# tangtang888/video-edge-ai-proxy

Measured on AMD Instinct MI355X. Metric: decoded FPS (whole node) + p50 VideoLatestImage latency, 256×1080p RTSP, higher is better.
Workload: dtype uint8 (BGR24 frames; bf16-capable consumer path)

## Files before the change

### csrc/bind_ext.h

```cpp
#pragma once
#include <pybind11/pybind11.h>

void bind_net(pybind11::module_& m);
void bind_mux(pybind11::module_& m);
void bind_hevc(pybind11::module_& m);
void bind_bus(pybind11::module_& m);
void bind_rpc(pybind11::module_& m);
void bind_dbk(pybind11::module_& m);
void bind_hevc_lf(pybind11::module_& m);
```

### csrc/bindings.cpp

```cpp
#include <malloc.h>

#include <pybind11/numpy.h>
#include <pybind11/pybind11.h>
#include <pybind11/stl.h>

#include "vep/hostprof.h"
#include "vep/avc.h"
#include "vep/avc_cavlc.h"
#include "vep/avc_recon.h"
#include "vep/bench_driver.h"
#include "vep/cabac.h"
#include "vep/codec.h"
#include "vep/gpu.h"
#include "vep/h264.h"
#include "vep/hevc_ctu.h"
#include "vep/hevc_dec.h"
#include "vep/hevc_kern.h"
#include "vep/jpeg.h"
#include "vep/scale.h"
#include "bind_ext.h"
#include "vep/runtime.h"
#include "vep/synth.h"

namespace py = pybind11;
// ... 2464 lines not shown
  m.def("letterbox_geometry", [](int src_w, int src_h, int size, bool even) {
    gpu::LetterboxDesc d{};
    d.src_w = src_w;
    d.src_h = src_h;
    gpu::fill_letterbox_geometry(d, size, even);
    return py::make_tuple(d.nw, d.nh, d.pad_x, d.pad_y);
  }, py::arg("src_w"), py::arg("src_h"), py::arg("size"), py::arg("even") = false);

  bind_net(m);
  bind_mux(m);
  bind_hevc(m);
  bind_bus(m);
  bind_rpc(m);
  bind_dbk(m);
  bind_hevc_lf(m);
}
```

### csrc/vep/avc.cpp

```cpp
#include "avc.h"

#include <immintrin.h>

#include <algorithm>
#include <array>

#include "avc_cavlc.h"
#include "avc_internal.h"
#include "fanout.h"

namespace vep::avc {

using h264::Pps;
using h264::Sps;


void MbNeighbours::reset(int wmbs, int hmbs, bool ring) {
  w_ = wmbs;
  h_ = hmbs;
  cur_ = -1;
  run_slice_ = ~0u;
  run_start_ = 0;
  announced_ = 0;
  const size_t n = size_t(wmbs) * hmbs;
// ... 1487 lines not shown
  if (par) {
    const int W = pic->wmbs, H = pic->hmbs;
    ColMotion* col_target = colb.col;
    FanOut::shared().run(nunits, [&](int k) {
      SliceUnit& u = *units_[size_t(k)];
      u.nb.reset(W, H, true);
      Picture& sh = u.shard;
      sh.wmbs = W;
      sh.hmbs = H;
      if (sh.mbs.size() != size_t(W) * H) sh.mbs.assign(size_t(W) * H, MbRec{});
      sh.coefs.clear();
      sh.mvs.clear();
      sh.wps.clear();
      sh.intra_mbs = sh.intra_res = sh.inter_mbs = 0;
      sh.deblock = false;
      sh.target = pic->target;
      sh.dpb_slots = pic->dpb_slots;
      sh.constrained_intra = pic->constrained_intra;
      sh.poc = pic->poc;
      sh.bd = pic->bd;
      sh.cf = pic->cf;
      sh.qp_bias = pic->qp_bias;
      sh.qpc_bias = pic->qpc_bias;
      u.colb.col = col_target;
      u.colb.set_uids(&u.uids);
      sh.colb = col_target ? &u.colb : nullptr;
      parse_slice_data(u.nb, sh, u.sh, *u.sps, *u.pps, u.rbsp.data(), u.rbsp.size(), u.bitpos, u.slice_idx, u.list);
#if defined(__x86_64__)
      _mm_sfence();
#endif
    });
    parallel_slices_run_ += u64(nunits);
    covered.assign(size_t(pic->nmbs()), 0);
    for (int k = 0; k < nunits; ++k) {
      SliceUnit& u = *units_[size_t(k)];
      const Picture& sh = u.shard;
      const u32 coef0 = u32(pic->coefs.size()), mv0 = u32(pic->mvs.size()), wp0 = u32(pic->wps.size());
      const u32 res0 = u32(pic->intra_res);
      pic->coefs.insert(pic->coefs.end(), sh.coefs.begin(), sh.coefs.end());
      pic->mvs.insert(pic->mvs.end(), sh.mvs.begin(), sh.mvs.end());
      pic->wps.insert(pic->wps.end(), sh.wps.begin(), sh.wps.end());
      pic->intra_mbs += sh.intra_mbs;
      pic->intra_res += sh.intra_res;
      pic->inter_mbs += sh.inter_mbs;
      pic->deblock |= sh.deblock;
      for (int mb = u.sh.first_mb; mb < pic->nmbs(); ++mb) {
        if (!u.nb.announced(mb)) continue;
        VEP_CHECK(!covered[size_t(mb)], "H.264: slices overlap");
        covered[size_t(mb)] = 1;
        MbRec m = sh.mbs[size_t(mb)];
        m.coef += coef0;
        if (m.kind == kSkip || m.kind == kInter) m.mv += mv0;
        if (m.flags & kMbWp) m.wp += wp0;
        if (m.res != kNoRes) m.res += res0;
        pic->mbs[size_t(mb)] = m;
      }
    }
  }
  int ncovered = 0;
  if (par)
// ... 19 lines not shown
      }
      for (auto& rf : m.ref) rf = u8(cs);
      m.mv = u32(pic->mvs.size());
      m.flags |= kMbMv16;
      pic->mvs.resize(pic->mvs.size() + 2, 0);
      ++pic->inter_mbs;
    } else {
      m.kind = kI16x16;
      m.i16_mode = 2;
      std::fill(std::begin(m.ref), std::end(m.ref), u8(0xFF));
      ++pic->intra_mbs;
    }
  }
  pic->info.coded_mbs = pic->nmbs() - missing;
  const u32 uid = next_uid_++;
  if (first.field_pic) {
    if (first.nal_ref_idc != 0)
      mark_field(first, *act_sps, pic->target >> 1, pic->poc, uid, second_field && pair_.ref, std::move(col_built));
    if (first.has_mmco5() && !second_field) {
      pic->poc = 0;
      pair_.frame_num = 0;
      pair_.poc[int(first.bottom_field)] = 0;
      pair_.boundary = true;
      pair_.hard = reorder_cur_ == 0;
    }
    if (second_field) close_pair(*pic);
  } else {
    if (first.nal_ref_idc != 0) {
      mark_references(first, *act_sps, pic->target, pic->poc, uid, std::move(col_built));
    }
// ... 41 lines not shown
      more = br.pos() < stop;
      ++mb;
    }
    return;
  }
  SliceEnv env;
  env.sh = &sh;
  env.sps = &sps;
  env.pps = &pps;
  env.slice = slice_idx;
  env.list[0] = &lists[0];
  env.list[1] = &lists[1];
  env.cur_poc = pic.poc;
  env.scaling = h264::resolve_scaling(sps, pps);
  env.field = sh.field_pic;
  decode_slice_generic(nb, pic, env, data, n, bitpos);
}

static inline void validate_mb(const Picture& p, const MbRec& m, bool written = false) {
  const size_t ncoef = p.coefs.size(), nmv = p.mvs.size();
  VEP_CHECK(m.kind <= kI8x8, "macroblock kind out of range");
  VEP_CHECK(p.cf == 2 || m.chroma_coded < 0x100, "chroma block mask out of range");
  VEP_CHECK(m.qp <= 51 + p.qp_bias && m.qpc <= 51 + p.qpc_bias && m.qpc2 <= 51 + p.qpc_bias,
            "macroblock QP out of range");
  if (m.kind == kIPcm) {
    const size_t ns = p.cf == 2 ? size_t(kPcmMaxSamples) : size_t(kPcmMbBytes);
    VEP_CHECK(size_t(m.coef) + (p.bd > 8 ? ns : ns / 2) <= ncoef, "I_PCM samples outside the pool");
    return;
  }
  const size_t nw = size_t(coef_words(m));
// ... 110 lines not shown
    stream_words(&col->b[size_t(mb) * 4], out, sizeof out);
    return;
  }
  ColMotion::Blk* out = &col->b[size_t(mb) * 16];
  for (int blk = 0; blk < 16; ++blk) {
    const int b8 = ((blk >> 3) << 1) | ((blk & 3) >> 1);
    const int l = st.ref[0][b8] >= 0 ? 0 : 1;
    const int ri = st.ref[l][b8];
    if (ri < 0) {
      out[blk] = ColMotion::Blk{{0, 0}, 0u, i8(-1)};
      continue;
    }
    out[blk] = ColMotion::Blk{{st.mv[l][blk][0], st.mv[l][blk][1]},
                              size_t(ri) < lu[size_t(l)].size() ? lu[size_t(l)][size_t(ri)] : 0u, i8(ri)};
  }
}

std::shared_ptr<ColMotion> build_col_motion(const MbNeighbours& nb, int wmbs, int hmbs,
                                            const std::vector<std::array<std::vector<u32>, 2>>& slice_uids,
                                            bool corners, Recycler<ColMotion>* pool) {
  auto col = pool ? pool->acquire([](ColMotion&) {}) : std::make_shared<ColMotion>();
  col->wmbs = wmbs;
  col->hmbs = hmbs;
  col->corners = corners;
  const int per = corners ? 4 : 16;
  col->b.resize(size_t(wmbs) * hmbs * size_t(per));
  static constexpr u8 kCorner[4] = {0, 3, 12, 15};
  for (int mb = 0; mb < wmbs * hmbs; ++mb) {
    const MbState& st = nb.at(mb);
    ColMotion::Blk* out = &col->b[size_t(mb) * size_t(per)];
// ... 237 lines not shown
  for (int l = 0; l < nl; ++l, out += per) {
    const i16* v = &s.mv[l][0][0];
    if (per == 2) {
      std::memcpy(out, v, 4);
    } else if (per == 8) {
      std::memcpy(out, v, 4);
      std::memcpy(out + 2, v + 4, 4);
      std::memcpy(out + 4, v + 16, 4);
      std::memcpy(out + 6, v + 20, 4);
    } else {
      std::memcpy(out, v, 64);
    }
  }
}

static inline void store_rec(MbRec* dst, const MbRec& m) {
  static_assert(sizeof(MbRec) % 8 == 0 && sizeof(ColMotion::Blk) * 4 % 8 == 0, "8-byte words");
  stream_words(dst, &m, sizeof(MbRec));
}

void store_skip_mb(Picture& pic, int mb, MbRec& m, const MbState& s) {
  m.coef = u32(pic.coefs.size());
  m.luma_coded = 0;
  m.chroma_coded = 0;
  m.wp = 0;
  m.res = kNoRes;
  store_motion(pic, m, s);
  ++pic.inter_mbs;
  if (!(m.dbk & 1)) pic.deblock = true;
  for (int k = 0; k < 4; ++k) {
    const int r0 = m.ref[k], r1 = m.ref1[k];
    VEP_CHECK((r0 != 0xFF || r1 != 0xFF) && (r0 == 0xFF || r0 < pic.dpb_slots) && (r1 == 0xFF || r1 < pic.dpb_slots) &&
                  (r1 == 0xFF || (m.flags & kMbL1)),
              "skipped macroblock reference slot outside the DPB");
  }
  VEP_CHECK(m.qp <= 51 + pic.qp_bias && m.qpc <= 51 + pic.qpc_bias && m.qpc2 <= 51 + pic.qpc_bias,
            "macroblock QP out of range");
  store_rec(&pic.mbs[size_t(mb)], m);
  if (pic.colb) pic.colb->store(mb, s);
}

void store_mb(Picture& pic, int mb, MbRec m, const MbState& s, const MbResidual* res, const u8* pcm,
              const WpEntry* wp) {
  m.coef = u32(pic.coefs.size());
  m.luma_coded = 0;
  m.chroma_coded = 0;
  if (m.kind == kIPcm) {
    VEP_CHECK(pcm, "I_PCM macroblock without samples");
    const size_t ns = pic.cf == 2 ? size_t(kPcmMaxSamples) : size_t(kPcmMbBytes);
    const size_t o = pic.coefs.size(), nb = pic.bd > 8 ? 2 * ns : ns;
    pic.coefs.resize(o + nb / 2);
    std::memcpy(pic.coefs.data() + o, pcm, nb);
  } else if (res && (res->luma | res->chroma)) {
    m.luma_coded = res->luma;
    m.chroma_coded = res->chroma;
    if (res->t8) m.flags |= kMbT8x8;
    const i16* grp[32];
    int ng = 0;
    if (res->t8) {
      for (int q = 0; q < 4; ++q)
        if ((res->luma >> ((q & 1) * 2 + (q >> 1) * 8)) & 1)
          for (int w = 0; w < 4; ++w) grp[ng++] = res->b8[q] + 16 * w;
    } else {
      for (u32 w = res->luma; w; w &= w - 1) grp[ng++] = res->blk[__builtin_ctz(w)];
    }
    for (u32 w = res->chroma; w; w &= w - 1) grp[ng++] = res->blk[16 + __builtin_ctz(w)];
    u16 mask[32];
    int nv = 0;
    for (int g = 0; g < ng; ++g) {
      mask[g] = nonzero_mask16(grp[g]);
      nv += __builtin_popcount(mask[g]);
    }
    const size_t o = pic.coefs.size();
    i16* out = pic.coefs.extend(size_t(ng + nv) + 8);
    std::memcpy(out, mask, size_t(ng) * sizeof(u16));
    i16* v = out + ng;
    for (int g = 0; g < ng; ++g) v = compact16(grp[g], mask[g], v);
    pic.coefs.resize(o + size_t(ng + nv));
  }
  m.mv = 0;
  m.wp = 0;
  m.flags &= u8(~(kMbMv8x8 | kMbMv16));
  if (m.kind == kSkip || m.kind == kInter) {
    store_motion(pic, m, s);
    if (wp && (m.flags & kMbWp)) {
      m.wp = u32(pic.wps.size());
      pic.wps.insert(pic.wps.end(), wp, wp + 4);
    } else {
      m.flags &= u8(~kMbWp);
    }
    ++pic.inter_mbs;
  } else if (m.kind == kIPcm) {
    ++pic.inter_mbs;
  } else {
    ++pic.intra_mbs;
  }
  m.res = is_intra(m.kind) && m.kind != kIPcm && (m.luma_coded | m.chroma_coded) ? u32(pic.intra_res++) : kNoRes;
  if (!(m.dbk & 1)) pic.deblock = true;
  validate_written_mb(pic, m);
// ... 356 lines not shown
```

### csrc/vep/avc.h

```cpp
#pragma once

#include <array>
#include <map>
#include <memory>

#include "hostmem.h"
#include "recycle.h"
#include "avc_recon.h"
#include "codec.h"

namespace vep::avc {

constexpr int kMaxDpbSlots = 34;

struct AuMeta {
  i64 pts = 0, dts = 0, arrival_ms = 0;
  i64 tag = 0;
  bool keyframe = false, corrupt = false;
};

struct OutFrame {
  int slot = -1;
  PictureInfo info;
  AuMeta au;
// ... 14 lines not shown
  int structure = 0;
  int bd = 8, qp_bias = 0, qpc_bias = 0;
  int cf = 1;
  bool second_field = false;
  bool constrained_intra = false;
  int intra_mbs = 0;
  int intra_res = 0;
  int inter_mbs = 0;
  bool deblock = false;
  bool idr = false;
  int poc = 0;
  PictureInfo info;
  AuMeta au;
  std::vector<OutFrame> outputs;
  ColBuild* colb = nullptr;

  int nmbs() const { return wmbs * hmbs; }
};
using PicturePtr = std::shared_ptr<const Picture>;

void validate(const Picture& p);

struct SliceHdr {
  int nal_type = 0, nal_ref_idc = 0;
  int first_mb = 0, slice_type = 0, pps_id = 0, frame_num = 0, idr_pic_id = 0;
  bool field_pic = false, bottom_field = false;
  int redundant_pic_cnt = 0;
  int poc_lsb = 0, delta_poc_bottom = 0, delta_poc[2] = {0, 0};
  bool direct_spatial = true;
  int num_ref_idx[2] = {1, 1};
// ... 279 lines not shown
  size_t index(int mb, int blk) const {
    return corners ? size_t(mb) * 4 + size_t(((blk >> 3) << 1) | ((blk & 3) >> 1)) : size_t(mb) * 16 + size_t(blk);
  }
};

struct ColBuild {
  ColMotion* col = nullptr;
  const std::array<std::vector<u32>, 2>* uids = nullptr;
  u32 uid_tab[2][32] = {};
  void set_uids(const std::array<std::vector<u32>, 2>* u) {
    uids = u;
    for (int l = 0; l < 2; ++l)
      for (size_t k = 0; k < 32; ++k) uid_tab[l][k] = u && k < (*u)[size_t(l)].size() ? (*u)[size_t(l)][k] : 0u;
  }
  void store(int mb, const MbState& st);
  void none(int mb);
};

struct RefPic {
  int slot = -1;
  int frame_num = 0;
  int frame_num_wrap = 0;
  bool long_term = false;
  int lt_idx = 0;
  int poc = 0;
  u32 uid = 0;
  std::shared_ptr<const ColMotion> col;
  u8 fields = 3;
  u8 lt_fields = 0;
  int poc_f[2] = {0, 0};
// ... 73 lines not shown
  bool field_mode_ = false;
  struct OpenPair {
    bool open = false;
    int slot = -1, frame_num = 0, bottom = 0;
    int poc[2] = {0, 0};
    bool ref = false, boundary = false, hard = false;
    u8 have = 0;
    OutFrame f;
  } pair_;
  void close_pair(Picture& pic);

 public:
  Decoder();
  ~Decoder();
  u64 parallel_slices_run() const { return parallel_slices_run_; }
  u64 mmco_ops[7] = {0, 0, 0, 0, 0, 0, 0};
  u64 list_mods = 0, long_term_marked = 0;
  u64 redundant_slices_skipped = 0;
};

void cpu_reconstruct(const Picture& pic, std::vector<HostSurface>& slots);
void weave_fields(const HostSurface& top, const HostSurface& bottom, HostSurface& frame);

struct MbLevels {
  int luma[16][16];
  int dc[16];
  int cdc[2][4];
  int cac[2][4][16];
  u16 lmask = 0;
  u8 cmask = 0;
// ... 7 lines not shown
      if (dc[k]) dcmask |= 1;
    for (int c = 0; c < 2; ++c)
      for (int b = 0; b < 4; ++b) {
        if (cdc[c][b]) dcmask |= u8(2 << c);
        for (int k = 0; k < 16; ++k)
          if (cac[c][b][k]) cmask |= u8(1u << (c * 4 + b));
      }
  }
};
struct MbResidual {
  i16 blk[32][16];
  i16 b8[4][64];
  u16 luma = 0;
  u16 chroma = 0;
  bool t8 = false;
};
void dequantize_mb(const MbLevels& lv, bool i16x16, int qp, int qpc, MbResidual& out);
void store_mb(Picture& pic, int mb, MbRec m, const MbState& s, const MbResidual* res, const u8* pcm,
              const WpEntry* wp = nullptr);
void store_skip_mb(Picture& pic, int mb, MbRec& m, const MbState& s);
void cpu_reconstruct_mb(const Picture& pic, int mb, std::vector<HostSurface>& slots);
void cpu_deblock(const Picture& pic, HostSurface& target);
void intra4x4_neighbours(const Picture& pic, int mb, int idx, const HostSurface& T, Intra4Nb& n);
void intra16_neighbours(const Picture& pic, int mb, const HostSurface& T, Intra16Nb& n);
void chroma_neighbours(const Picture& pic, int mb, int c, const HostSurface& T, IntraChromaNb& n);
void intra8x8_neighbours(const Picture& pic, int mb, int q, const HostSurface& T, int* f, bool& has_top,
                         bool& has_left);

class StreamEncoder {
 public:
  virtual ~StreamEncoder() = default;
  virtual std::shared_ptr<AccessUnit> next() = 0;
  virtual const HostSurface& reconstruction() const = 0;
  virtual const HostSurface& source() const = 0;
  virtual i64 last_pts() const = 0;
// ... 93 lines not shown
```

### csrc/vep/avc_internal.h

```cpp
#pragma once

#include <array>

#include "avc.h"
#include "bits.h"

namespace vep::avc {

struct SliceEnv {
  const SliceHdr* sh = nullptr;
  const h264::Sps* sps = nullptr;
  const h264::Pps* pps = nullptr;
  int slice = 0;
  const std::vector<ListEntry>* list[2] = {nullptr, nullptr};
  int cur_poc = 0;
  h264::ScalingLists scaling;
  bool field = false;
};

void decode_slice_generic(MbNeighbours& nb, Picture& pic, const SliceEnv& env, const u8* data, size_t n,
                          size_t bitpos);

WpEntry wp_entry(const SliceEnv& env, int r0, int r1);

std::shared_ptr<ColMotion> build_col_motion(const MbNeighbours& nb, int wmbs, int hmbs,
                                            const std::vector<std::array<std::vector<u32>, 2>>& slice_uids,
                                            bool corners, Recycler<ColMotion>* pool = nullptr);

void predict_inter(const std::vector<HostSurface>& slots, const MbRec& m, const i16* mv0, const i16* mv1,
                   const WpEntry* wp, int mx, int my, int* py, int (*pc)[128], int structure = 0);

struct MbDesc {
// ... 54 lines not shown
```

### csrc/vep/avc_mb.cpp

```cpp
#include <algorithm>
#include <memory>
#include <cstddef>
#include <cstring>

#include "avc_cabac.h"
#include "avc_cavlc.h"
#include "avc_internal.h"

namespace vep::avc {

namespace {

struct Dequant {
  int ls4[6][6][16];
  int ls8[2][6][64];
  explicit Dequant(const h264::ScalingLists& sl) {
    for (int l = 0; l < 6; ++l)
      for (int m = 0; m < 6; ++m)
        for (int k = 0; k < 16; ++k) {
          const int pos = kZigzag4x4[k];
          ls4[l][m][pos] = int(sl.l4[l][k]) * norm_adjust(m, pos >> 2, pos & 3);
        }
    for (int l = 0; l < 2; ++l)
      for (int m = 0; m < 6; ++m)
// ... 48 lines not shown
    cf_ = sps_.chroma_format_idc;
    nbc_ = cf_ == 2 ? 8 : 4;
    weighted_ = (type_ == h264::kP && pps_.weighted_pred) || (type_ == h264::kB && pps_.weighted_bipred_idc != 0);
    implicit_ = type_ == h264::kB && pps_.weighted_bipred_idc == 2;
    for (int l = 0; l < 2; ++l) {
      std::fill(std::begin(slot_[l]), std::end(slot_[l]), u8(0xFF));
      if (const auto* lst = env_.list[l])
        for (size_t k = 0; k < lst->size() && k + 1 < std::size(slot_[l]); ++k)
          if ((*lst)[k].slot >= 0) slot_[l][k + 1] = u8((*lst)[k].slot);
    }
    for (int q = 0; q < 52 + qpbd_ && q < int(std::size(qpc_tab_[0])); ++q) {
      qpc_tab_[0][q] = u8(chroma_qp_bd(q - qpbd_, pps_.chroma_qp_index_offset, qpbdc_) + qpbdc_);
      qpc_tab_[1][q] = u8(chroma_qp_bd(q - qpbd_, pps_.second_chroma_qp_index_offset, qpbdc_) + qpbdc_);
    }
    fast_direct_ = !kWrite && type_ == h264::kB && sh_.direct_spatial && sps_.direct_8x8 && !weighted_;
  }

  Bits* br = nullptr;
  BitWriter* bw = nullptr;
  Bins* bins = nullptr;
  cabac::Decoder* cabac = nullptr;
  cabac::Encoder* cenc = nullptr;
  const MbDesc* want = nullptr;
  int prev_qpd_nz = 0;

  int qp() const { return qp_; }

  int ue(u32 v) {
    if constexpr (kWrite) {
      bw->ue(v);
// ... 46 lines not shown
    s.kind = kSkip;
    s.skip = 1;
    s.qp = u8(qp_ + qpbd_);
    MbResidual res;
    res.luma = 0;
    res.chroma = 0;
    if (type_ == h264::kP) {
      s.ref[0][0] = s.ref[0][1] = s.ref[0][2] = s.ref[0][3] = 0;
      need_ref(0, 0);
      int mv[2];
      nb_.pskip_mv(mb, mv);
      for (auto& v : s.mv[0]) {
        v[0] = i16(mv[0]);
        v[1] = i16(mv[1]);
      }
    } else {
      s.direct16 = 1;
      s.direct8 = 0xF;
      if (fast_direct_) direct16_spatial(mb, s);
      else direct(mb, s, 0xF);
    }
    prev_qpd_nz = 0;
    if (!weighted_ && !kWrite) emit_skip(mb, s);
    else emit(mb, s, res, 0, 0, nullptr);
  }

  void coded_mb(int mb, bool fresh) {
    MbState& s = nb_.at(mb);
    if (fresh) {
      s = MbState{};
      s.slice = u16(env_.slice);
      nb_.begin(mb);
    } else if constexpr (!kWrite) {
      std::memset(static_cast<void*>(s.mv), 0, sizeof s.mv);
    }
    int mbt = read_mb_type(mb, kWrite ? want->mb_type : 0);
    int itype = -1;
    if (type_ == h264::kI) {
      itype = mbt;
    } else if (type_ == h264::kP) {
      VEP_CHECK(mbt <= 30, "bad P mb_type");
      if (mbt >= 5) itype = mbt - 5;
    } else {
      VEP_CHECK(mbt <= 48, "bad B mb_type");
      if (mbt >= 23) itype = mbt - 23;
    }
    VEP_CHECK(itype <= 25, "bad intra mb_type");
    MbResidual res;
    res.luma = 0;
    res.chroma = 0;
// ... 339 lines not shown
  }
  static void set_mv(MbState& s, int list, const Part& p, int mx, int my) {
    VEP_CHECK(mx >= -32768 && mx <= 32767 && my >= -32768 && my <= 32767, "motion vector out of range");
    for (int y = p.y4; y < p.y4 + p.h4; ++y)
      for (int x = p.x4; x < p.x4 + p.w4; ++x) {
        s.mv[list][y * 4 + x][0] = i16(mx);
        s.mv[list][y * 4 + x][1] = i16(my);
      }
  }

  bool inter_pred(int mb, MbState& s, int mbt) {
    const bool b = type_ == h264::kB;
    if (b && mbt == 0) {
      s.direct16 = 1;
      s.direct8 = 0xF;
      if (fast_direct_) direct16_spatial(mb, s);
      else direct(mb, s, 0xF);
      return true;
    }
    if ((!b && mbt <= 2) || (b && mbt <= 21)) {
      Part parts[2];
      int np;
      u8 pred[2];
      int shape;
      if (!b) {
        shape = mbt;
        pred[0] = pred[1] = 1;
      } else {
        shape = mbt <= 3 ? 0 : ((mbt & 1) ? 2 : 1);
        pred[0] = kBPart[mbt][0];
        pred[1] = kBPart[mbt][1];
      }
// ... 233 lines not shown
    if (zero) ref[0] = ref[1] = 0;
    u32 pv[2];
    for (int l = 0; l < 2; ++l) {
      if (ref[l] >= 0) need_ref(l, ref[l]);
      const bool use = ref[l] >= 0 && !zero;
      pv[l] = use ? (u32(u16(mvp[l][0])) | u32(u16(mvp[l][1])) << 16) : 0u;
      std::memset(s.ref[l], ref[l], 4);
    }
    const ColMotion::Blk* cb = &dcol_->b[size_t(mb) * 4];
    u32 v8[2][4];
    for (int b8 = 0; b8 < 4; ++b8) {
      const bool col_zero = !dcol_long_ && cb[b8].ref == 0 && cb[b8].mv[0] >= -1 && cb[b8].mv[0] <= 1 &&
                            cb[b8].mv[1] >= -1 && cb[b8].mv[1] <= 1;
      for (int l = 0; l < 2; ++l) v8[l][b8] = (ref[l] == 0 && col_zero) ? 0u : pv[l];
    }
    for (int l = 0; l < 2; ++l) {
      u32 row[2][4];
      for (int h = 0; h < 2; ++h) {
        row[h][0] = row[h][1] = v8[l][2 * h];
        row[h][2] = row[h][3] = v8[l][2 * h + 1];
      }
      u8* mv = reinterpret_cast<u8*>(&s.mv[l][0][0]);
      for (int y = 0; y < 4; ++y) std::memcpy(mv + 16 * y, row[y >> 1], 16);
    }
  }

  WpEntry weights(int r0, int r1) { return wp_entry(env_, r0, r1); }

  int cbf_luma_inc(int mb, int blk, bool intra) {
    auto cond = [&](int m, int nblk) -> int {
// ... 54 lines not shown
      } else {
        read_residual_block_cb(*br, nc, n, [&](int k, int l) {
          lv[k] = l;
          nzpos[t++] = u8(k);
        });
        return t;
      }
    }
  }

  void residual(int mb, MbState& s, MbResidual& res, int cbp_luma, int cbp_chroma, int qp, bool intra) {
    const int ly = intra ? 0 : 3;
    const int q6 = qp / 6, qm = qp % 6;
    int lv[64];
    u8 nzp[64];
    if (s.kind == kI16x16) {
      const int inc = kCabac ? cbf_dc_inc(mb, 0, true) : 0;
      const int nc = kCabac ? 0 : nb_.nc_luma(mb, 0);
      int dcy[16] = {};
      const int tdc = read_block(kCatLumaDc, inc, nc, 16, lv, nzp, kWrite ? want->dc : nullptr);
      if (tdc > 0) {
        s.cbf_dc |= 1;
        int c[16] = {};
        for (int j = 0; j < tdc; ++j) c[scan4_[nzp[j]]] = lv[nzp[j]];
        hadamard4x4(c);
        const int ls = dq_.ls4[ly][qm][0];
        for (int k = 0; k < 16; ++k)
          dcy[k] = qp >= 36 ? c[k] * ls * (1 << (q6 - 6)) : (c[k] * ls + (1 << (5 - q6))) >> (6 - q6);
      }
      for (int idx = 0; idx < 16; ++idx) {
        const int r = blk_to_raster(idx);
        i16* d = res.blk[r];
        bool nz = dcy[r] != 0;
        std::memset(d, 0, 16 * sizeof(i16));
        d[0] = sat16(dcy[r]);
        if (cbp_luma) {
          const int binc = kCabac ? cbf_luma_inc(mb, r, true) : 0;
          const int bnc = kCabac ? 0 : nb_.nc_luma(mb, r);
          const int tc = read_block(kCatLumaAc, binc, bnc, 15, lv, nzp, kWrite ? want->ac[r] : nullptr);
          for (int j = 0; j < tc; ++j) {
            const int k = nzp[j];
            const int pos = scan4_[k + 1];
            const int v = scale4(lv[k], dq_.ls4[ly][qm][pos], qp);
            d[pos] = sat16(v);
            nz |= v != 0;
          }
          s.tc[r] = u8(tc);
          if (tc) s.cbf |= u16(1u << r);
        }
        if (nz) res.luma |= u16(1u << r);
      }
    } else if (s.t8x8) {
      res.t8 = true;
      const int l8 = intra ? 0 : 1;
      for (int b8 = 0; b8 < 4; ++b8) {
        if (!((cbp_luma >> b8) & 1)) continue;
        i16* d = res.b8[b8];
        std::memset(d, 0, 64 * sizeof(i16));
        bool nz = false;
        int total = 0;
        auto put = [&](int k, int level) {
          const int pos = scan8_[k];
          const int v = scale8(level, dq_.ls8[l8][qm][pos], qp);
          d[pos] = sat16(v);
          nz |= v != 0;
        };
        if constexpr (kCabac) {
          total = read_block(kCatLuma8x8, -1, 0, 64, lv, nzp, kWrite ? want->l8[b8] : nullptr);
          for (int j = 0; j < total; ++j) put(nzp[j], lv[nzp[j]]);
          for (u16 w = b8_blocks(b8); w; w &= w - 1) s.tc[__builtin_ctz(w)] = u8(std::min(total, 16));
        } else {
          for (int i4 = 0; i4 < 4; ++i4) {
            const int r = blk_to_raster(b8 * 4 + i4);
            int part[16] = {};
            if constexpr (kWrite)
              for (int k = 0; k < 16; ++k) part[k] = want->l8[b8][4 * k + i4];
            const int tc = read_block(kCatLuma4x4, 0, nb_.nc_luma(mb, r), 16, lv, nzp, part);
            s.tc[r] = u8(tc);
            total += tc;
            for (int j = 0; j < tc; ++j) put(4 * nzp[j] + i4, lv[nzp[j]]);
          }
        }
        if (total) {
          s.cbf |= b8_blocks(b8);
          nz8_ |= b8_blocks(b8);
        }
        if (nz) res.luma |= b8_blocks(b8);
      }
    } else {
      for (int idx = 0; idx < 16; ++idx) {
        const int r = blk_to_raster(idx);
        if (!((cbp_luma >> (idx >> 2)) & 1)) continue;
        const int binc = kCabac ? cbf_luma_inc(mb, r, intra) : 0;
        const int bnc = kCabac ? 0 : nb_.nc_luma(mb, r);
        const int tc = read_block(kCatLuma4x4, binc, bnc, 16, lv, nzp, kWrite ? want->ac[r] : nullptr);
        s.tc[r] = u8(tc);
        if (!tc) continue;
        s.cbf |= u16(1u << r);
        i16* d = res.blk[r];
        std::memset(d, 0, 16 * sizeof(i16));
        bool nz = false;
        for (int j = 0; j < tc; ++j) {
          const int k = nzp[j];
          const int pos = scan4_[k];
          const int v = scale4(lv[k], dq_.ls4[ly][qm][pos], qp);
          d[pos] = sat16(v);
          nz |= v != 0;
        }
        if (nz) res.luma |= u16(1u << r);
      }
    }
    if (cbp_chroma) {
      const int qpc[2] = {chroma_qp_bd(qp - qpbd_, pps_.chroma_qp_index_offset, qpbdc_) + qpbdc_,
                          chroma_qp_bd(qp - qpbd_, pps_.second_chroma_qp_index_offset, qpbdc_) + qpbdc_};
      const int nbc = nbc_;
      int dcv[2][8] = {};
      for (int c = 0; c < 2; ++c) {
        const int inc = kCabac ? cbf_dc_inc(mb, 1 + c, intra) : 0;
        int v8[8];
        const int t = read_block(kCatChromaDc, inc, cf_ == 2 ? -2 : -1, nbc, v8, nzp, kWrite ? want->cdc[c] : nullptr);
        if (t > 0) {
          s.cbf_dc |= u8(2 << c);
          int u[8] = {0, 0, 0, 0, 0, 0, 0, 0};
          for (int j = 0; j < t; ++j) u[nzp[j]] = v8[nzp[j]];
          if (cf_ == 2) {
            const int qpdc = qpc[c] + 3;
            chroma422_dc(u, qpdc, dq_.ls4[ly + 1 + c][qpdc % 6][0], dcv[c]);
          } else {
            const int f[4] = {u[0] + u[1] + u[2] + u[3], u[0] - u[1] + u[2] - u[3], u[0] + u[1] - u[2] - u[3],
                              u[0] - u[1] - u[2] + u[3]};
            const int ls = dq_.ls4[ly + 1 + c][qpc[c] % 6][0];
            for (int b = 0; b < 4; ++b) dcv[c][b] = ((f[b] * ls) * (1 << (qpc[c] / 6))) >> 5;
          }
        }
      }
      for (int c = 0; c < 2; ++c) {
        const int lc = ly + 1 + c;
        for (int b = 0; b < nbc; ++b) {
          i16* d = res.blk[16 + c * nbc + b];
          bool nz = dcv[c][b] != 0;
          std::memset(d, 0, 16 * sizeof(i16));
          d[0] = sat16(dcv[c][b]);
          if (cbp_chroma & 2) {
            const int binc = kCabac ? cbf_cac_inc(mb, c, b, intra) : 0;
            const int bnc = kCabac ? 0 : nb_.nc_chroma(mb, c, b, nbc);
            const int tc = read_block(kCatChromaAc, binc, bnc, 15, lv, nzp, kWrite ? want->cac[c][b] : nullptr);
            s.tcc[c][b] = u8(tc);
            if (tc) s.cbf_cac[c] |= u8(1u << b);
            for (int j = 0; j < tc; ++j) {
              const int k = nzp[j];
              const int pos = scan4_[k + 1];
              const int v = scale4(lv[k], dq_.ls4[lc][qpc[c] % 6][pos], qpc[c]);
              d[pos] = sat16(v);
              nz |= v != 0;
            }
          }
          if (nz) res.chroma |= u16(1u << (c * nbc + b));
        }
      }
    }
    if constexpr (!kCabac && !kWrite) VEP_CHECK(!br->overrun(), "slice data overrun");
  }

  void emit(int mb, const MbState& s, const MbResidual& res, int i16_mode, int chroma_mode, const u8* pcm) {
    MbRec m{};
    m.kind = s.kind;
    m.qp = u8(s.kind == kIPcm ? qpbd_ : s.qp);
    VEP_CHECK(m.qp < std::size(qpc_tab_[0]), "macroblock QP out of range");
    m.qpc = qpc_tab_[0][m.qp];
    m.qpc2 = qpc_tab_[1][m.qp];
    m.i16_mode = u8(i16_mode);
    m.chroma_mode = u8(chroma_mode);
// ... 29 lines not shown
      for (int r = 0; r < 16; ++r) m.i4[r >> 1] |= u8(s.i4[r] << ((r & 1) * 4));
    if (s.kind == kI8x8)
      for (int b8 = 0; b8 < 4; ++b8) m.i4[b8 >> 1] |= u8(s.i4[(b8 & 1) * 2 + (b8 >> 1) * 8] << ((b8 & 1) * 4));
    WpEntry wp[4];
    bool use_wp = false;
    if (weighted_ && !is_intra(s.kind)) {
      for (int k = 0; k < 4; ++k) {
        wp[k] = weights(s.ref[0][k], s.ref[1][k]);
        const WpEntry& e = wp[k];
        for (int c = 0; c < 3; ++c)
          use_wp |= !(e.lwd[c] == 0 && e.w0[c] == 1 && e.w1[c] == 1 && e.o[c] == 0) &&
                    !(e.w0[c] == (1 << e.lwd[c]) && e.w1[c] == (1 << e.lwd[c]) && e.o[c] == 0);
      }
      if (use_wp) m.flags |= kMbWp;
    }
    store_mb(pic_, mb, m, s, &res, pcm, use_wp ? wp : nullptr);
  }

  void emit_skip(int mb, const MbState& s) {
    MbRec m{};
    m.kind = kSkip;
    m.qp = s.qp;
    VEP_CHECK(m.qp < std::size(qpc_tab_[0]), "macroblock QP out of range");
    m.qpc = qpc_tab_[0][m.qp];
    m.qpc2 = qpc_tab_[1][m.qp];
    m.dbk = u8((sh_.disable_deblocking == 1 ? 1 : 0) | (sh_.disable_deblocking == 2 ? 2 : 0));
    m.alpha_off = i8(sh_.alpha_off);
    m.beta_off = i8(sh_.beta_off);
    m.slice = s.slice;
    bool l1 = false;
    for (int k = 0; k < 4; ++k) {
      m.ref[k] = slot_[0][s.ref[0][k] + 1];
      m.ref1[k] = slot_[1][s.ref[1][k] + 1];
      l1 |= s.ref[1][k] >= 0;
    }
    m.flags = l1 ? kMbL1 : 0;
    nz8_ = 0;
    store_skip_mb(pic_, mb, m, s);
  }

  MbNeighbours& nb_;
  Picture& pic_;
  const SliceEnv& env_;
  const SliceHdr& sh_;
  const h264::Pps& pps_;
  const h264::Sps& sps_;
  const Dequant& dq_;
  const u8* scan4_;
  const u8* scan8_;
  int type_ = 0;
  int qp_ = 26;
  bool weighted_ = false, implicit_ = false;
  u16 nz8_ = 0;
  u8 slot_[2][33];
  u8 qpc_tab_[2][96];
  bool fast_direct_ = false;
  const ColMotion* dcol_ = nullptr;
  bool dcol_long_ = false;
};

}

WpEntry wp_entry(const SliceEnv& env, int r0, int r1) {
  const SliceHdr& sh = *env.sh;
  const bool implicit = sh.type() == h264::kB && env.pps->weighted_bipred_idc == 2;
  WpEntry e{};
  for (int c = 0; c < 3; ++c) {
    e.w0[c] = e.w1[c] = 1;
    e.o[c] = 0;
    e.lwd[c] = 0;
  }
  if (implicit) {
    if (r0 < 0 || r1 < 0) return e;
// ... 184 lines not shown
```

Baseline: 8444.

## Add fast CABAC paths for skip MBs, shared motion, uniform colocated stores, sparse coefs

Adds several fast paths to the CPU H.264 CABAC slice parser. Skipped and spatial-direct macroblocks get a cached MbRec template and packed motion words. Identical consecutive motion vectors reuse one pool entry, and uniform colocated motion is written directly. Residual blocks track nonzero coefficient masks during dequantization instead of memsetting and rescanning them. It also adds counters, a generic_paths toggle and a Python probe binding for equivalence checking, at the cost of more code paths that must match the generic output exactly.

```diff
diff --git a/csrc/bind_ext.h b/csrc/bind_ext.h
--- a/csrc/bind_ext.h
+++ b/csrc/bind_ext.h
@@ -8,3 +8,4 @@
 void bind_rpc(pybind11::module_& m);
 void bind_dbk(pybind11::module_& m);
 void bind_hevc_lf(pybind11::module_& m);
+void bind_parse(pybind11::module_& m);
diff --git a/csrc/bind_parse.cpp b/csrc/bind_parse.cpp
--- /dev/null
+++ b/csrc/bind_parse.cpp
@@ -0,0 +1,91 @@
+#include <pybind11/numpy.h>
+#include <pybind11/pybind11.h>
+#include <pybind11/stl.h>
+
+#include <cstddef>
+#include <cstring>
+#include <memory>
+#include <string>
+#include <vector>
+
+#include "bind_ext.h"
+#include "vep/avc.h"
+#include "vep/avc_probe.h"
+#include "vep/codec.h"
+
+namespace py = pybind11;
+using namespace vep;
+
+namespace {
+
+py::dict picture_dict(const avc::Picture& p, const avc::ColMotion* col) {
+  py::dict d;
+  const size_t n = size_t(p.nmbs());
+  d["wmbs"] = p.wmbs;
+  d["hmbs"] = p.hmbs;
+  d["type"] = std::string(1, p.info.pict_type);
+  d["structure"] = p.structure;
+  py::array_t<u8> recs({n, sizeof(avc::MbRec)});
+  if (n) std::memcpy(recs.mutable_data(), p.mbs.data(), n * sizeof(avc::MbRec));
+  d["recs"] = recs;
+  py::array_t<avc::i16> motion({n, size_t(2), size_t(16), size_t(2)});
+  for (size_t mb = 0; mb < n; ++mb)
+    avc::probe::expand_motion(p, int(mb), reinterpret_cast<i16(*)[16][2]>(motion.mutable_data() + mb * 64));
+  d["motion"] = motion;
+  py::array_t<avc::i16> coefs(p.coefs.size());
+  if (p.coefs.size()) std::memcpy(coefs.mutable_data(), p.coefs.data(), p.coefs.size() * sizeof(i16));
+  d["coefs"] = coefs;
+  d["mv_pool_entries"] = p.mvs.size();
+  if (col) {
+    const size_t nb = col->b.size();
+    py::array_t<avc::i16> mv({nb, size_t(2)});
+    py::array_t<u32> pid(nb);
+    py::array_t<avc::i8> ref(nb);
+    for (size_t k = 0; k < nb; ++k) {
+      mv.mutable_data()[2 * k] = col->b[k].mv[0];
+      mv.mutable_data()[2 * k + 1] = col->b[k].mv[1];
+      pid.mutable_data()[k] = col->b[k].pid;
+      ref.mutable_data()[k] = col->b[k].ref;
+    }
+    py::dict c;
+    c["corners"] = col->corners;
+    c["mv"] = mv;
+    c["pid"] = pid;
+    c["ref"] = ref;
+    d["col"] = c;
+  } else {
+    d["col"] = py::none();
+  }
+  py::dict f;
+  f["skip_header"] = p.fast.skip_header;
+  f["shared_mv"] = p.fast.shared_mv;
+  f["col_uniform"] = p.fast.col_uniform;
+  f["sparse"] = p.fast.sparse;
+  d["fast"] = f;
+  return d;
+}
+
+}
+
+void bind_parse(py::module_& m) {
+  m.attr("AVC_MBREC_MV_OFFSET") = offsetof(avc::MbRec, mv);
+  m.def(
+      "avc_parse_pictures",
+      [](const std::vector<std::shared_ptr<AccessUnit>>& aus, bool generic) {
+        avc::Decoder dec;
+        dec.generic_paths = generic;
+        dec.keep_last_col = true;
+        py::list out;
+        for (const auto& au : aus) {
+          VEP_CHECK(au != nullptr, "avc_parse_pictures: null access unit");
+          size_t nal = 0;
+          do {
+            dec.last_col.reset();
+            avc::PicturePtr pic = dec.parse(*au, 0, &nal);
+            out.append(picture_dict(*pic, dec.last_col.get()));
+          } while (nal < au->nals.size());
+        }
+        return out;
+      },
+      py::arg("aus"), py::arg("generic") = false);
+}
diff --git a/csrc/bindings.cpp b/csrc/bindings.cpp
--- a/csrc/bindings.cpp
+++ b/csrc/bindings.cpp
@@ -2502,4 +2502,5 @@
   bind_rpc(m);
   bind_dbk(m);
   bind_hevc_lf(m);
+  bind_parse(m);
 }
diff --git a/csrc/vep/avc.cpp b/csrc/vep/avc.cpp
--- a/csrc/vep/avc.cpp
+++ b/csrc/vep/avc.cpp
@@ -1525,6 +1525,7 @@
       sh.wps.clear();
       sh.intra_mbs = sh.intra_res = sh.inter_mbs = 0;
       sh.deblock = false;
+      sh.fast = Picture::FastPaths{};
       sh.target = pic->target;
       sh.dpb_slots = pic->dpb_slots;
       sh.constrained_intra = pic->constrained_intra;
@@ -1555,6 +1556,10 @@
       pic->intra_res += sh.intra_res;
       pic->inter_mbs += sh.inter_mbs;
       pic->deblock |= sh.deblock;
+      pic->fast.skip_header += sh.fast.skip_header;
+      pic->fast.shared_mv += sh.fast.shared_mv;
+      pic->fast.col_uniform += sh.fast.col_uniform;
+      pic->fast.sparse += sh.fast.sparse;
       for (int mb = u.sh.first_mb; mb < pic->nmbs(); ++mb) {
         if (!u.nb.announced(mb)) continue;
         VEP_CHECK(!covered[size_t(mb)], "H.264: slices overlap");
@@ -1604,6 +1609,7 @@
   }
   pic->info.coded_mbs = pic->nmbs() - missing;
   const u32 uid = next_uid_++;
+  if (keep_last_col) last_col = col_built;
   if (first.field_pic) {
     if (first.nal_ref_idc != 0)
       mark_field(first, *act_sps, pic->target >> 1, pic->poc, uid, second_field && pair_.ref, std::move(col_built));
@@ -1675,6 +1681,7 @@
   env.cur_poc = pic.poc;
   env.scaling = h264::resolve_scaling(sps, pps);
   env.field = sh.field_pic;
+  env.generic = generic_paths;
   decode_slice_generic(nb, pic, env, data, n, bitpos);
 }
 
@@ -1815,6 +1822,13 @@
     out[blk] = ColMotion::Blk{{st.mv[l][blk][0], st.mv[l][blk][1]},
                               size_t(ri) < lu[size_t(l)].size() ? lu[size_t(l)][size_t(ri)] : 0u, i8(ri)};
   }
+}
+
+void ColBuild::store_uniform(int mb, int l, int ri, const u32 w[4]) {
+  ColMotion::Blk out[4];
+  const u32 pid = uid_tab[l][ri & 31];
+  for (int k = 0; k < 4; ++k) out[k] = ColMotion::Blk{{i16(u16(w[k])), i16(u16(w[k] >> 16))}, pid, i8(ri)};
+  stream_words(&col->b[size_t(mb) * 4], out, sizeof out);
 }
 
 std::shared_ptr<ColMotion> build_col_motion(const MbNeighbours& nb, int wmbs, int hmbs,
@@ -2082,6 +2096,40 @@
   }
 }
 
+static inline void store_motion_words(Picture& pic, MbRec& m, const MotionWords& mw) {
+  const int nl = (m.flags & kMbL1) ? 2 : 1;
+  MotionShare& sh = *mw.share;
+#if defined(__AVX2__)
+  const __m256i w = _mm256_loadu_si256(reinterpret_cast<const __m256i*>(mw.w));
+  const u32 eq0 = u32(_mm256_movemask_epi8(_mm256_cmpeq_epi32(w, _mm256_shuffle_epi32(w, 0))));
+  const bool one = (eq0 | (nl == 2 ? 0u : 0xFFFF0000u)) == 0xFFFFFFFFu;
+  const bool eqw = u32(_mm256_movemask_epi8(_mm256_cmpeq_epi32(
+                       w, _mm256_loadu_si256(reinterpret_cast<const __m256i*>(sh.w))))) == 0xFFFFFFFFu;
+#else
+  bool one = true, eqw = true;
+  for (int l = 0; l < 2; ++l)
+    for (int k = 0; k < 4; ++k) {
+      one &= l >= nl || mw.w[l][k] == mw.w[l][0];
+      eqw &= sh.w[l][k] == mw.w[l][k];
+    }
+#endif
+  const u8 f = u8((m.flags & kMbL1) | (one ? kMbMv16 : kMbMv8x8));
+  m.flags |= f;
+  const int per = one ? 1 : 4;
+  if (sh.valid & (sh.flags == f) & eqw) {
+    m.mv = sh.off;
+    ++pic.fast.shared_mv;
+    return;
+  }
+  m.mv = u32(pic.mvs.size());
+  i16* out = pic.mvs.extend(size_t(2 * per * nl));
+  for (int l = 0; l < nl; ++l) std::memcpy(out + 2 * per * l, mw.w[l], size_t(per) * 4);
+  std::memcpy(sh.w, mw.w, sizeof sh.w);
+  sh.valid = true;
+  sh.flags = f;
+  sh.off = m.mv;
+}
+
 static inline void store_rec(MbRec* dst, const MbRec& m) {
   static_assert(sizeof(MbRec) % 8 == 0 && sizeof(ColMotion::Blk) * 4 % 8 == 0, "8-byte words");
   stream_words(dst, &m, sizeof(MbRec));
@@ -2108,8 +2156,25 @@
   if (pic.colb) pic.colb->store(mb, s);
 }
 
+void store_skip_words(Picture& pic, int mb, MbRec& m, const MbState& s, const MotionWords& mw, int l, int ri) {
+  m.coef = u32(pic.coefs.size());
+  store_motion_words(pic, m, mw);
+  ++pic.inter_mbs;
+  ++pic.fast.skip_header;
+  if (!(m.dbk & 1)) pic.deblock = true;
+  store_rec(&pic.mbs[size_t(mb)], m);
+  if (ColBuild* cb = pic.colb) {
+    if (cb->uids && cb->col->corners) {
+      cb->store_uniform(mb, l, ri, mw.w[l]);
+      ++pic.fast.col_uniform;
+    } else {
+      cb->store(mb, s);
+    }
+  }
+}
+
 void store_mb(Picture& pic, int mb, MbRec m, const MbState& s, const MbResidual* res, const u8* pcm,
-              const WpEntry* wp) {
+              const WpEntry* wp, const MotionWords* mw) {
   m.coef = u32(pic.coefs.size());
   m.luma_coded = 0;
   m.chroma_coded = 0;
@@ -2124,20 +2189,43 @@
     m.chroma_coded = res->chroma;
     if (res->t8) m.flags |= kMbT8x8;
     const i16* grp[32];
-    int ng = 0;
-    if (res->t8) {
-      for (int q = 0; q < 4; ++q)
-        if ((res->luma >> ((q & 1) * 2 + (q >> 1) * 8)) & 1)
-          for (int w = 0; w < 4; ++w) grp[ng++] = res->b8[q] + 16 * w;
+    u16 mask[32];
+    int ng = 0, nv = 0;
+    if (res->masked) {
+      if (res->t8) {
+        for (int q = 0; q < 4; ++q)
+          if ((res->luma >> ((q & 1) * 2 + (q >> 1) * 8)) & 1)
+            for (int w = 0; w < 4; ++w) {
+              mask[ng] = u16(res->gmask8[q] >> (16 * w));
+              grp[ng++] = res->b8[q] + 16 * w;
+            }
+      } else {
+        for (u32 w = res->luma; w; w &= w - 1) {
+          const int r = __builtin_ctz(w);
+          mask[ng] = res->gmask[r];
+          grp[ng++] = res->blk[r];
+        }
+      }
+      for (u32 w = res->chroma; w; w &= w - 1) {
+        const int k = 16 + __builtin_ctz(w);
+        mask[ng] = res->gmask[k];
+        grp[ng++] = res->blk[k];
+      }
+      for (int g = 0; g < ng; ++g) nv += __builtin_popcount(mask[g]);
+      ++pic.fast.sparse;
     } else {
-      for (u32 w = res->luma; w; w &= w - 1) grp[ng++] = res->blk[__builtin_ctz(w)];
-    }
-    for (u32 w = res->chroma; w; w &= w - 1) grp[ng++] = res->blk[16 + __builtin_ctz(w)];
-    u16 mask[32];
-    int nv = 0;
-    for (int g = 0; g < ng; ++g) {
-      mask[g] = nonzero_mask16(grp[g]);
-      nv += __builtin_popcount(mask[g]);
+      if (res->t8) {
+        for (int q = 0; q < 4; ++q)
+          if ((res->luma >> ((q & 1) * 2 + (q >> 1) * 8)) & 1)
+            for (int w = 0; w < 4; ++w) grp[ng++] = res->b8[q] + 16 * w;
+      } else {
+        for (u32 w = res->luma; w; w &= w - 1) grp[ng++] = res->blk[__builtin_ctz(w)];
+      }
+      for (u32 w = res->chroma; w; w &= w - 1) grp[ng++] = res->blk[16 + __builtin_ctz(w)];
+      for (int g = 0; g < ng; ++g) {
+        mask[g] = nonzero_mask16(grp[g]);
+        nv += __builtin_popcount(mask[g]);
+      }
     }
     const size_t o = pic.coefs.size();
     i16* out = pic.coefs.extend(size_t(ng + nv) + 8);
@@ -2150,7 +2238,8 @@
   m.wp = 0;
   m.flags &= u8(~(kMbMv8x8 | kMbMv16));
   if (m.kind == kSkip || m.kind == kInter) {
-    store_motion(pic, m, s);
+    if (mw) store_motion_words(pic, m, *mw);
+    else store_motion(pic, m, s);
     if (wp && (m.flags & kMbWp)) {
       m.wp = u32(pic.wps.size());
       pic.wps.insert(pic.wps.end(), wp, wp + 4);
diff --git a/csrc/vep/avc.h b/csrc/vep/avc.h
--- a/csrc/vep/avc.h
+++ b/csrc/vep/avc.h
@@ -52,6 +52,12 @@
   AuMeta au;
   std::vector<OutFrame> outputs;
   ColBuild* colb = nullptr;
+  struct FastPaths {
+    u32 skip_header = 0;
+    u32 shared_mv = 0;
+    u32 col_uniform = 0;
+    u32 sparse = 0;
+  } fast;
 
   int nmbs() const { return wmbs * hmbs; }
 };
@@ -361,6 +367,7 @@
       for (size_t k = 0; k < 32; ++k) uid_tab[l][k] = u && k < (*u)[size_t(l)].size() ? (*u)[size_t(l)][k] : 0u;
   }
   void store(int mb, const MbState& st);
+  void store_uniform(int mb, int l, int ri, const u32 w[4]);
   void none(int mb);
 };
 
@@ -464,6 +471,9 @@
   Decoder();
   ~Decoder();
   u64 parallel_slices_run() const { return parallel_slices_run_; }
+  bool generic_paths = false;
+  bool keep_last_col = false;
+  std::shared_ptr<const ColMotion> last_col;
   u64 mmco_ops[7] = {0, 0, 0, 0, 0, 0, 0};
   u64 list_mods = 0, long_term_marked = 0;
   u64 redundant_slices_skipped = 0;
@@ -501,11 +511,25 @@
   u16 luma = 0;
   u16 chroma = 0;
   bool t8 = false;
+  bool masked = false;
+  u16 gmask[32];
+  u64 gmask8[4];
+};
+struct MotionShare {
+  bool valid = false;
+  u8 flags = 0;
+  u32 off = 0;
+  u32 w[2][4] = {};
+};
+struct MotionWords {
+  const u32 (*w)[4];
+  MotionShare* share;
 };
 void dequantize_mb(const MbLevels& lv, bool i16x16, int qp, int qpc, MbResidual& out);
 void store_mb(Picture& pic, int mb, MbRec m, const MbState& s, const MbResidual* res, const u8* pcm,
-              const WpEntry* wp = nullptr);
+              const WpEntry* wp = nullptr, const MotionWords* mw = nullptr);
 void store_skip_mb(Picture& pic, int mb, MbRec& m, const MbState& s);
+void store_skip_words(Picture& pic, int mb, MbRec& m, const MbState& s, const MotionWords& mw, int l, int ri);
 void cpu_reconstruct_mb(const Picture& pic, int mb, std::vector<HostSurface>& slots);
 void cpu_deblock(const Picture& pic, HostSurface& target);
 void intra4x4_neighbours(const Picture& pic, int mb, int idx, const HostSurface& T, Intra4Nb& n);
diff --git a/csrc/vep/avc_internal.h b/csrc/vep/avc_internal.h
--- a/csrc/vep/avc_internal.h
+++ b/csrc/vep/avc_internal.h
@@ -16,6 +16,7 @@
   int cur_poc = 0;
   h264::ScalingLists scaling;
   bool field = false;
+  bool generic = false;
 };
 
 void decode_slice_generic(MbNeighbours& nb, Picture& pic, const SliceEnv& env, const u8* data, size_t n,
diff --git a/csrc/vep/avc_mb.cpp b/csrc/vep/avc_mb.cpp
--- a/csrc/vep/avc_mb.cpp
+++ b/csrc/vep/avc_mb.cpp
@@ -86,6 +86,14 @@
       qpc_tab_[1][q] = u8(chroma_qp_bd(q - qpbd_, pps_.second_chroma_qp_index_offset, qpbdc_) + qpbdc_);
     }
     fast_direct_ = !kWrite && type_ == h264::kB && sh_.direct_spatial && sps_.direct_8x8 && !weighted_;
+    fast_ = kCabac && !kWrite && !env.generic && !env.field && !weighted_;
+    masked_ = kCabac && !kWrite && !env.generic;
+    tmpl_.kind = kSkip;
+    tmpl_.dbk = u8((sh_.disable_deblocking == 1 ? 1 : 0) | (sh_.disable_deblocking == 2 ? 2 : 0));
+    tmpl_.alpha_off = i8(sh_.alpha_off);
+    tmpl_.beta_off = i8(sh_.beta_off);
+    tmpl_.slice = u16(env_.slice);
+    tmpl_.res = kNoRes;
   }
 
   Bits* br = nullptr;
@@ -162,6 +170,9 @@
         v[0] = i16(mv[0]);
         v[1] = i16(mv[1]);
       }
+      dw_[0][0] = dw_[0][1] = dw_[0][2] = dw_[0][3] = u32(u16(mv[0])) | u32(u16(mv[1])) << 16;
+      dref_[0] = 0;
+      dref_[1] = -1;
     } else {
       s.direct16 = 1;
       s.direct8 = 0xF;
@@ -169,7 +180,8 @@
       else direct(mb, s, 0xF);
     }
     prev_qpd_nz = 0;
-    if (!weighted_ && !kWrite) emit_skip(mb, s);
+    if (fast_ && (type_ == h264::kP || fast_direct_)) emit_skip_words(mb, s);
+    else if (!weighted_ && !kWrite) emit_skip(mb, s);
     else emit(mb, s, res, 0, 0, nullptr);
   }
 
@@ -182,6 +194,7 @@
     } else if constexpr (!kWrite) {
       std::memset(static_cast<void*>(s.mv), 0, sizeof s.mv);
     }
+    direct_words_ = false;
     int mbt = read_mb_type(mb, kWrite ? want->mb_type : 0);
     int itype = -1;
     if (type_ == h264::kI) {
@@ -551,8 +564,12 @@
     if (b && mbt == 0) {
       s.direct16 = 1;
       s.direct8 = 0xF;
-      if (fast_direct_) direct16_spatial(mb, s);
-      else direct(mb, s, 0xF);
+      if (fast_direct_) {
+        direct16_spatial(mb, s);
+        direct_words_ = fast_;
+      } else {
+        direct(mb, s, 0xF);
+      }
       return true;
     }
     if ((!b && mbt <= 2) || (b && mbt <= 21)) {
@@ -816,6 +833,9 @@
                             cb[b8].mv[1] >= -1 && cb[b8].mv[1] <= 1;
       for (int l = 0; l < 2; ++l) v8[l][b8] = (ref[l] == 0 && col_zero) ? 0u : pv[l];
     }
+    std::memcpy(dw_, v8, sizeof dw_);
+    dref_[0] = ref[0];
+    dref_[1] = ref[1];
     for (int l = 0; l < 2; ++l) {
       u32 row[2][4];
       for (int h = 0; h < 2; ++h) {
@@ -900,6 +920,8 @@
     const int q6 = qp / 6, qm = qp % 6;
     int lv[64];
     u8 nzp[64];
+    const bool masked = masked_;
+    res.masked = masked;
     if (s.kind == kI16x16) {
       const int inc = kCabac ? cbf_dc_inc(mb, 0, true) : 0;
       const int nc = kCabac ? 0 : nb_.nc_luma(mb, 0);
@@ -917,8 +939,8 @@
       for (int idx = 0; idx < 16; ++idx) {
         const int r = blk_to_raster(idx);
         i16* d = res.blk[r];
-        bool nz = dcy[r] != 0;
-        std::memset(d, 0, 16 * sizeof(i16));
+        u32 gm = dcy[r] != 0;
+        if (!masked) std::memset(d, 0, 16 * sizeof(i16));
         d[0] = sat16(dcy[r]);
         if (cbp_luma) {
           const int binc = kCabac ? cbf_luma_inc(mb, r, true) : 0;
@@ -929,12 +951,13 @@
             const int pos = scan4_[k + 1];
             const int v = scale4(lv[k], dq_.ls4[ly][qm][pos], qp);
             d[pos] = sat16(v);
-            nz |= v != 0;
+            gm |= u32(v != 0) << pos;
           }
           s.tc[r] = u8(tc);
           if (tc) s.cbf |= u16(1u << r);
         }
-        if (nz) res.luma |= u16(1u << r);
+        res.gmask[r] = u16(gm);
+        if (gm) res.luma |= u16(1u << r);
       }
     } else if (s.t8x8) {
       res.t8 = true;
@@ -942,14 +965,14 @@
       for (int b8 = 0; b8 < 4; ++b8) {
         if (!((cbp_luma >> b8) & 1)) continue;
         i16* d = res.b8[b8];
-        std::memset(d, 0, 64 * sizeof(i16));
-        bool nz = false;
+        if (!masked) std::memset(d, 0, 64 * sizeof(i16));
+        u64 gm = 0;
         int total = 0;
         auto put = [&](int k, int level) {
           const int pos = scan8_[k];
           const int v = scale8(level, dq_.ls8[l8][qm][pos], qp);
           d[pos] = sat16(v);
-          nz |= v != 0;
+          gm |= u64(v != 0) << pos;
         };
         if constexpr (kCabac) {
           total = read_block(kCatLuma8x8, -1, 0, 64, lv, nzp, kWrite ? want->l8[b8] : nullptr);
@@ -971,7 +994,8 @@
           s.cbf |= b8_blocks(b8);
           nz8_ |= b8_blocks(b8);
         }
-        if (nz) res.luma |= b8_blocks(b8);
+        res.gmask8[b8] = gm;
+        if (gm) res.luma |= b8_blocks(b8);
       }
     } else {
       for (int idx = 0; idx < 16; ++idx) {
@@ -984,16 +1008,17 @@
         if (!tc) continue;
         s.cbf |= u16(1u << r);
         i16* d = res.blk[r];
-        std::memset(d, 0, 16 * sizeof(i16));
-        bool nz = false;
+        if (!masked) std::memset(d, 0, 16 * sizeof(i16));
+        u32 gm = 0;
         for (int j = 0; j < tc; ++j) {
           const int k = nzp[j];
           const int pos = scan4_[k];
           const int v = scale4(lv[k], dq_.ls4[ly][qm][pos], qp);
           d[pos] = sat16(v);
-          nz |= v != 0;
-        }
-        if (nz) res.luma |= u16(1u << r);
+          gm |= u32(v != 0) << pos;
+        }
+        res.gmask[r] = u16(gm);
+        if (gm) res.luma |= u16(1u << r);
       }
     }
     if (cbp_chroma) {
@@ -1024,8 +1049,8 @@
         const int lc = ly + 1 + c;
         for (int b = 0; b < nbc; ++b) {
           i16* d = res.blk[16 + c * nbc + b];
-          bool nz = dcv[c][b] != 0;
-          std::memset(d, 0, 16 * sizeof(i16));
+          u32 gm = dcv[c][b] != 0;
+          if (!masked) std::memset(d, 0, 16 * sizeof(i16));
           d[0] = sat16(dcv[c][b]);
           if (cbp_chroma & 2) {
             const int binc = kCabac ? cbf_cac_inc(mb, c, b, intra) : 0;
@@ -1038,10 +1063,11 @@
               const int pos = scan4_[k + 1];
               const int v = scale4(lv[k], dq_.ls4[lc][qpc[c] % 6][pos], qpc[c]);
               d[pos] = sat16(v);
-              nz |= v != 0;
+              gm |= u32(v != 0) << pos;
             }
           }
-          if (nz) res.chroma |= u16(1u << (c * nbc + b));
+          res.gmask[16 + c * nbc + b] = u16(gm);
+          if (gm) res.chroma |= u16(1u << (c * nbc + b));
         }
       }
     }
@@ -1101,7 +1127,8 @@
       }
       if (use_wp) m.flags |= kMbWp;
     }
-    store_mb(pic_, mb, m, s, &res, pcm, use_wp ? wp : nullptr);
+    const MotionWords mw{dw_, &share_};
+    store_mb(pic_, mb, m, s, &res, pcm, use_wp ? wp : nullptr, direct_words_ ? &mw : nullptr);
   }
 
   void emit_skip(int mb, const MbState& s) {
@@ -1124,6 +1151,34 @@
     m.flags = l1 ? kMbL1 : 0;
     nz8_ = 0;
     store_skip_mb(pic_, mb, m, s);
+  }
+
+  void emit_skip_words(int mb, const MbState& s) {
+    if (int(s.qp) != tmpl_qp_) {
+      VEP_CHECK(s.qp < std::size(qpc_tab_[0]), "macroblock QP out of range");
+      tmpl_.qp = s.qp;
+      tmpl_.qpc = qpc_tab_[0][s.qp];
+      tmpl_.qpc2 = qpc_tab_[1][s.qp];
+      VEP_CHECK(tmpl_.qp <= 51 + pic_.qp_bias && tmpl_.qpc <= 51 + pic_.qpc_bias && tmpl_.qpc2 <= 51 + pic_.qpc_bias,
+                "macroblock QP out of range");
+      tmpl_qp_ = s.qp;
+    }
+    if (dref_[0] != tmpl_ref_[0] || dref_[1] != tmpl_ref_[1]) {
+      const int r0 = slot_[0][dref_[0] + 1], r1 = slot_[1][dref_[1] + 1];
+      VEP_CHECK((r0 != 0xFF || r1 != 0xFF) && (r0 == 0xFF || r0 < pic_.dpb_slots) && (r1 == 0xFF || r1 < pic_.dpb_slots) &&
+                    (r1 == 0xFF || dref_[1] >= 0),
+                "skipped macroblock reference slot outside the DPB");
+      std::memset(tmpl_.ref, r0, 4);
+      std::memset(tmpl_.ref1, r1, 4);
+      tmpl_l1_ = dref_[1] >= 0 ? kMbL1 : 0;
+      tmpl_ref_[0] = dref_[0];
+      tmpl_ref_[1] = dref_[1];
+    }
+    MbRec m = tmpl_;
+    m.flags = tmpl_l1_;
+    nz8_ = 0;
+    const int l = dref_[0] >= 0 ? 0 : 1;
+    store_skip_words(pic_, mb, m, s, MotionWords{dw_, &share_}, l, dref_[l]);
   }
 
   MbNeighbours& nb_;
@@ -1144,6 +1199,16 @@
   bool fast_direct_ = false;
   const ColMotion* dcol_ = nullptr;
   bool dcol_long_ = false;
+  bool fast_ = false;
+  bool masked_ = false;
+  bool direct_words_ = false;
+  u32 dw_[2][4] = {};
+  int dref_[2] = {-1, -1};
+  MbRec tmpl_{};
+  int tmpl_qp_ = -1;
+  int tmpl_ref_[2] = {-2, -2};
+  u8 tmpl_l1_ = 0;
+  MotionShare share_;
 };
 
 }
diff --git a/csrc/vep/avc_probe.h b/csrc/vep/avc_probe.h
--- /dev/null
+++ b/csrc/vep/avc_probe.h
@@ -0,0 +1,58 @@
+#pragma once
+
+#include <cstring>
+#include <string>
+
+#include "avc.h"
+
+namespace vep::avc::probe {
+
+inline void expand_motion(const Picture& p, int mb, i16 out[2][16][2]) {
+  std::memset(out, 0, sizeof(i16) * 2 * 16 * 2);
+  const MbRec& m = p.mbs[size_t(mb)];
+  if (m.kind != kSkip && m.kind != kInter) return;
+  const int nl = (m.flags & kMbL1) ? 2 : 1;
+  const i16* base = p.mvs.data() + size_t(m.mv);
+  for (int l = 0; l < nl; ++l)
+    for (int b = 0; b < 16; ++b) {
+      const int o = mv_sub(m.flags, l, b);
+      out[l][b][0] = base[o];
+      out[l][b][1] = base[o + 1];
+    }
+}
+
+inline std::string compare(const Picture& a, const Picture& b) {
+  if (a.wmbs != b.wmbs || a.hmbs != b.hmbs || a.mbs.size() != b.mbs.size()) return "picture size";
+  if (a.coefs.size() != b.coefs.size() ||
+      (a.coefs.size() && std::memcmp(a.coefs.data(), b.coefs.data(), a.coefs.size() * sizeof(i16)) != 0))
+    return "coefficient pool";
+  if (a.wps.size() != b.wps.size() ||
+      (a.wps.size() && std::memcmp(a.wps.data(), b.wps.data(), a.wps.size() * sizeof(WpEntry)) != 0))
+    return "weight pool";
+  if (a.intra_mbs != b.intra_mbs || a.inter_mbs != b.inter_mbs || a.intra_res != b.intra_res || a.deblock != b.deblock)
+    return "picture counters";
+  for (int mb = 0; mb < a.nmbs(); ++mb) {
+    MbRec x = a.mbs[size_t(mb)], y = b.mbs[size_t(mb)];
+    x.mv = y.mv = 0;
+    if (std::memcmp(&x, &y, sizeof x) != 0) return "record of MB " + std::to_string(mb);
+    i16 ma[2][16][2], mb2[2][16][2];
+    expand_motion(a, mb, ma);
+    expand_motion(b, mb, mb2);
+    if (std::memcmp(ma, mb2, sizeof ma) != 0) return "motion of MB " + std::to_string(mb);
+  }
+  return "";
+}
+
+inline std::string compare(const ColMotion* a, const ColMotion* b) {
+  if (!a || !b) return a == b ? "" : "colocated motion present in one parse only";
+  if (a->wmbs != b->wmbs || a->hmbs != b->hmbs || a->corners != b->corners || a->b.size() != b->b.size())
+    return "colocated motion shape";
+  for (size_t k = 0; k < a->b.size(); ++k) {
+    const ColMotion::Blk &x = a->b[k], &y = b->b[k];
+    if (x.mv[0] != y.mv[0] || x.mv[1] != y.mv[1] || x.pid != y.pid || x.ref != y.ref)
+      return "colocated motion entry " + std::to_string(k);
+  }
+  return "";
+}
+
+}
```

Result: no change. 8442 (-0.0%).
